# HeewoongNoh/DOSTransformer

Hardware: AMD Instinct MI355X
Metric: crystals/sec training throughput (Phonon DOS, hidden=128) (higher is better)
Workload: dtype f32; 1 GPU; phonon_h128_b64: phonon DOSTransformer layers=3 transformer=2 hidden=128, 64 crystals/GPU, full train step (fwd+loss+bwd+AdamW), 8 distinct pre-collated HBM-resident batches; global_batch=64, parallelism=dp1, launch=replay

## Files before the change

### dostransformer_amd/_lib.py

```python
from __future__ import annotations

import ctypes as C
import os
from typing import Optional

_HERE = os.path.dirname(os.path.abspath(__file__))


def from_environ(name: str, default: str = "") -> str:
    return os.environ.get(name, default)


LIB_PATH = from_environ("DOSX_LIB") or os.path.join(_HERE, "csrc", "libdosx.so")

c_float_p = C.POINTER(C.c_float)
c_int_p = C.POINTER(C.c_int32)
BIG = 1 << 30


class DosxUnavailable(RuntimeError):
    pass


class DosxError(RuntimeError):
# ... 42 lines not shown
        ("pro_gamma", C.c_void_p), ("pro_beta", C.c_void_p), ("pro_alpha", C.c_void_p), ("pro_stats", C.c_void_p),
        ("slab", C.c_void_p), ("slab_bias", C.c_void_p),
        ("nsplit", C.c_int32), ("accumulate", C.c_int32),
        ("dst", C.c_void_p), ("dst_bias", C.c_void_p), ("counters", C.c_void_p), ("ldd", C.c_int32),
    ]


class ReduceJob(C.Structure):
    _fields_ = [("src", C.c_void_p), ("dst", C.c_void_p), ("nsplit", C.c_int32), ("stride", C.c_int32),
                ("count", C.c_int32), ("accumulate", C.c_int32)]


class Attn(C.Structure):
    _fields_ = [
        ("Sq", C.c_int32), ("Bq", C.c_int32), ("Nk", C.c_int32), ("Bk", C.c_int32), ("H", C.c_int32),
        ("q_stride_s", C.c_int32), ("q_stride_b", C.c_int32), ("flags", C.c_int32),
        ("x", C.c_void_p), ("kvhat", C.c_void_p), ("gamma0", C.c_void_p), ("beta0", C.c_void_p),
        ("out", C.c_void_p), ("probs", C.c_void_p), ("qstats", C.c_void_p), ("out_stats", C.c_void_p),
        ("dout", C.c_void_p), ("dx", C.c_void_p), ("dscores", C.c_void_p), ("dkvhat", C.c_void_p),
        ("dkv_accumulate", C.c_int32),
        ("partials_q", C.c_void_p), ("partials_kv", C.c_void_p), ("drop_mask", C.c_void_p), ("dkv_part", C.c_void_p), ("dkv_cnt", C.c_void_p),
        ("ln1_gamma", C.c_void_p), ("ln1_beta", C.c_void_p), ("ln1_out", C.c_void_p),
        ("key_ptr", C.c_void_p),
    ]


class FfnBwd(C.Structure):
    _fields_ = [
        ("M", C.c_int32), ("H", C.c_int32),
        ("dy", C.c_void_p), ("lddy", C.c_int32),
        ("h", C.c_void_p), ("ldh", C.c_int32),
        ("x", C.c_void_p), ("ldx", C.c_int32),
        ("stats", C.c_void_p),
        ("gamma", C.c_void_p),
        ("w1", C.c_void_p), ("w2", C.c_void_p),
        ("dh", C.c_void_p), ("lddh", C.c_int32),
        ("dx", C.c_void_p), ("lddx", C.c_int32),
        ("partials", C.c_void_p), ("partial_ld", C.c_int32),
        ("fin_gamma", C.c_void_p), ("fin_xhat", C.c_void_p), ("fin_rstd", C.c_void_p),
        ("fin_dy", C.c_void_p),
        ("fin_ddos", C.c_void_p), ("fin_w", C.c_void_p), ("fin_beta", C.c_void_p),
        ("fin_S", C.c_int32), ("fin_Bq", C.c_int32),
        ("att_x", C.c_void_p), ("att_ldxin", C.c_int32),
        ("att_kvhat", C.c_void_p), ("att_gamma0", C.c_void_p), ("att_beta0", C.c_void_p),
        ("att_probs", C.c_void_p), ("att_qstats", C.c_void_p), ("att_mask", C.c_void_p),
        ("att_dxin", C.c_void_p), ("att_lddxin", C.c_int32),
        ("att_partials_q", C.c_void_p), ("att_partials_kv", C.c_void_p), ("att_dkv_part", C.c_void_p), ("att_dkv_cnt", C.c_void_p),
        ("att_dkvhat", C.c_void_p), ("att_dkv_accumulate", C.c_int32),
        ("att_Nk", C.c_int32), ("att_Bk", C.c_int32), ("att_Bq", C.c_int32), ("att_Sq", C.c_int32), ("att_qs", C.c_int32), ("att_qb", C.c_int32),
    ]


class Ffn(C.Structure):
    _fields_ = [
        ("M", C.c_int32), ("H", C.c_int32),
        ("x", C.c_void_p), ("ldx", C.c_int32),
        ("stats", C.c_void_p),
        ("gamma", C.c_void_p), ("beta", C.c_void_p),
        ("w1", C.c_void_p), ("b1", C.c_void_p),
        ("w2", C.c_void_p), ("b2", C.c_void_p),
        ("h", C.c_void_p), ("ldh", C.c_int32),
        ("out", C.c_void_p), ("ldo", C.c_int32),
        ("fin_gamma", C.c_void_p), ("fin_beta", C.c_void_p),
        ("fin_xhat", C.c_void_p), ("fin_rstd", C.c_void_p),
        ("fin_w", C.c_void_p), ("fin_b", C.c_void_p), ("fin_dos", C.c_void_p),
        ("fin_S", C.c_int32), ("fin_Bq", C.c_int32),
        ("att_kvhat", C.c_void_p), ("att_gamma0", C.c_void_p), ("att_beta0", C.c_void_p), ("att_mask", C.c_void_p),
        ("att_probs", C.c_void_p), ("att_qstats", C.c_void_p), ("att_x1", C.c_void_p), ("att_st1", C.c_void_p),
        ("att_Nk", C.c_int32), ("att_Bk", C.c_int32), ("att_Bq", C.c_int32), ("att_Sq", C.c_int32),
        ("att_qs", C.c_int32), ("att_qb", C.c_int32), ("att_ldx1", C.c_int32), ("att_aligned", C.c_int32),
        ("att_key_ptr", C.c_void_p),
    ]
# ... 349 lines not shown
```

### dostransformer_amd/csrc/ffn.hip

```cpp
#include <stdlib.h>

#include "common.h"
#include "mma16.h"

typedef int v4i32 __attribute__((ext_vector_type(4)));

#ifdef DOSX_STAMPS
__device__ unsigned long long dosx_ffn_stamp_buf[64];
extern "C" int dosx_debug_read_ffn_stamps(unsigned long long* host64) {
  return (int)hipMemcpyFromSymbol(host64, HIP_SYMBOL(dosx_ffn_stamp_buf), sizeof(unsigned long long) * 64);
}
#define FSTAMP(slot) do { if (threadIdx.x == 0 && blockIdx.x == 0) dosx_ffn_stamp_buf[(slot)] = __builtin_amdgcn_s_memtime(); } while (0)
#define FSTAMP_S(slot) do { if (threadIdx.x == 256 && blockIdx.x == 0) dosx_ffn_stamp_buf[32 + (slot)] = __builtin_amdgcn_s_memtime(); } while (0)
#else
#define FSTAMP(slot) do { } while (0)
#define FSTAMP_S(slot) do { } while (0)
#endif

namespace {

constexpr int FBN = 128;

__device__ __forceinline__ void ffn_att_row(const DosxFfn& a, float* __restrict__ Xs, const int LDX, const int lr, const int m0,
                                            const int lane) {
// ... 606 lines not shown
  ffn_fwd_body<HALF, KB, ATT>(a, sm);
}

constexpr int FFN_MULTI_MAX = 2;
struct FfnMulti {
  DosxFfn d[FFN_MULTI_MAX];
  int n;
};
template <bool HALF, int KB, int ATT>
__global__ __launch_bounds__(512) void ffn_fwd_multi_kernel(const FfnMulti A) {
  DOSX_SET_MAIN_PRIO();
  extern __shared__ __align__(16) float sm[];
  ffn_fwd_body<HALF, KB, ATT>(A.d[0], sm);
  asm volatile("s_waitcnt vmcnt(0)" ::: "memory");
  __syncthreads();
  ffn_fwd_body<HALF, KB, ATT>(A.d[1], sm);
}


struct AttBwdSm {
  float *Os, *Ds, *Ql, *Sp, *Ks, *Sc, *Ss, *Ps2, *Pp;
};

__device__ __forceinline__ void ffn_dkv_reduce(const DosxFfnBwd& a, const int nqt, const int bk, float* __restrict__ Pp, const int tid) {
  const int lane = tid & 63, q16 = lane & 15, slot = tid >> 4;
  const int H = a.H, Nk = a.att_Nk, rep = a.att_Bq / a.att_Bk, ngroups = (Nk + 15) / 16;
  const int np = rep * nqt;
  const UDiv dnqt(nqt);
  const size_t pstride = (size_t)Nk * H;
  const __amdgpu_buffer_rsrc_t rP = __builtin_amdgcn_make_buffer_rsrc((void*)a.att_dkv_part, 0, 0x7fffffff, 0x00020000);
  float4 g0[2], d[2][2], kh[2][2], d0[2][2];
  bool jv[2];
  size_t krow[2];
#pragma unroll
  for (int k = 0; k < 2; ++k) g0[k] = ld4(a.att_gamma0 + ((q16 * 4 + 64 * k) < H ? (q16 * 4 + 64 * k) : 0));
#pragma unroll
  for (int p = 0; p < 2; ++p) {
    const int j = slot + 32 * p;
    jv[p] = j < Nk;
    krow[p] = ((size_t)(jv[p] ? j : 0) * a.att_Bk + bk) * H;
#pragma unroll
    for (int k = 0; k < 2; ++k) {
      const int c = q16 * 4 + 64 * k, cc = c < H ? c : 0;
      kh[p][k] = ld4(a.att_kvhat + krow[p] + cc);
      d0[p][k] = a.att_dkv_accumulate ? ld4(a.att_dkvhat + krow[p] + cc) : f4zero();
      d[p][k] = f4zero();
    }
  }
  for (int p0 = 0; p0 < np; p0 += 4) {
    float4 v[2][4][2];
#pragma unroll
    for (int p = 0; p < 2; ++p)
#pragma unroll
      for (int u = 0; u < 4; ++u) {
        const int pi = min(p0 + u, np - 1), i = dnqt.div(pi), t = pi - i * nqt;
        const size_t off = ((size_t)(bk + i * a.att_Bk) * nqt + t) * pstride + (size_t)(jv[p] ? slot + 32 * p : 0) * H;
#pragma unroll
        for (int k = 0; k < 2; ++k) {
          const int c = q16 * 4 + 64 * k;
          v[p][u][k] = __builtin_bit_cast(float4, __builtin_amdgcn_raw_buffer_load_b128(rP, (uint32_t)((off + (c < H ? c : 0)) * 4), 0, 16));
        }
      }
#pragma unroll
    for (int p = 0; p < 2; ++p)
#pragma unroll
      for (int u = 0; u < 4; ++u)
        if (p0 + u < np) {
#pragma unroll
          for (int k = 0; k < 2; ++k) d[p][k] = f4add(d[p][k], v[p][u][k]);
        }
  }
#pragma unroll
  for (int p = 0; p < 2; ++p)
#pragma unroll
    for (int k = 0; k < 2; ++k) {
      const int c = q16 * 4 + 64 * k;
      float4 pg = f4zero(), pb = f4zero();
      if (jv[p] && c < H) {
        pg = make_float4(d[p][k].x * kh[p][k].x, d[p][k].y * kh[p][k].y, d[p][k].z * kh[p][k].z, d[p][k].w * kh[p][k].w);
        pb = d[p][k];
        st4(a.att_dkvhat + krow[p] + c, make_float4(d[p][k].x * g0[k].x + d0[p][k].x, d[p][k].y * g0[k].y + d0[p][k].y,
                                                    d[p][k].z * g0[k].z + d0[p][k].z, d[p][k].w * g0[k].w + d0[p][k].w));
      }
      st4(Pp + (slot + 32 * p) * 256 + c, pg);
      st4(Pp + (slot + 32 * p) * 256 + 128 + c, pb);
    }
  __syncthreads();
  const UDiv dH(H), d2H(2 * H);
  for (int o = tid; o < ngroups * 2 * H; o += 512) {
    const int grp = d2H.div(o), c = o - grp * 2 * H;
    const int hi = dH.div(c), col = hi * 128 + (c - hi * H);
    float t = 0.f;
#pragma unroll
    for (int sl = 0; sl < 16; ++sl) t += Pp[(grp * 16 + sl) * 256 + col];
    a.att_partials_kv[((size_t)bk * ngroups + grp) * 2 * H + c] = t;
  }
}

struct AttBwdRegs {
  float4 g0[2], b0[2], xr[2], kr[4];
  float mean, rstd, pr[4], mk[4];
};
template <int R>
__device__ __forceinline__ void ffn_att_bwd_prefetch(const DosxFfnBwd& a, AttBwdRegs& q, const int al_s0, const int al_bq, const int tid) {
  const int H = a.H, lane = tid & 63, wave = tid >> 6, q16 = lane & 15, g4 = lane >> 4;
  const int Nk = a.att_Nk, NkP = (Nk + 15) & ~15, Sq = a.att_Sq, bk = al_bq % a.att_Bk;
  const int lr = wave * 4 + g4;
  const int s = min(al_s0 + (lr < R ? lr : 0), Sq - 1);
  const size_t orow = (size_t)s * a.att_Bq + al_bq;
  const float* xrow = a.att_x + ((size_t)s * a.att_qs + (size_t)al_bq * a.att_qb) * a.att_ldxin;
#pragma unroll
  for (int k = 0; k < 2; ++k) {
    const int c = q16 * 4 + 64 * k, cc = c < H ? c : 0;
    q.g0[k] = ld4(a.att_gamma0 + cc); q.b0[k] = ld4(a.att_beta0 + cc);
    q.xr[k] = c < H ? ld4(xrow + c) : f4zero();
  }
  q.mean = a.att_qstats[2 * orow]; q.rstd = a.att_qstats[2 * orow + 1];
  const size_t prow_ = ((size_t)al_bq * Sq + s) * Nk;
#pragma unroll
// ... 34 lines not shown
  const float mean = q.mean, rstd = q.rstd;
#pragma unroll
  for (int jj = 0; jj < 4; ++jj) { pr[jj] = q.pr[jj]; mk[jj] = q.mk[jj]; }
  {
    const int h4 = H >> 2;
    const UDiv dh4(h4);
#pragma unroll
    for (int i = 0; i < 4; ++i) {
      const int e = tid + 512 * i, j = dh4.div(e), c = (e - j * h4) * 4;
      if (e < NkP * h4) st4(L.Ks + j * LDK + c, q.kr[i]);
    }
  }
  FSTAMP(17);
  float cq = 0.f;
  if (rowok) {
    float t = 0.f;
#pragma unroll
    for (int k = 0; k < 2; ++k) {
      go[k] = f4zero();
      if (!on[k]) continue;
      go[k] = ld4(L.Os + lr * LDK + q16 * 4 + 64 * k);
      st4(L.Ds + lr * LDK + q16 * 4 + 64 * k, make_float4(go[k].x * g0[k].x, go[k].y * g0[k].y, go[k].z * g0[k].z, go[k].w * g0[k].w));
      t += (go[k].x * b0[k].x + go[k].y * b0[k].y) + (go[k].z * b0[k].z + go[k].w * b0[k].w);
    }
    if (a.att_mask) cq = row16_sum(t);
  }
  FSTAMP(18);
  __syncthreads();
  FSTAMP(19);
  const int nctS = NkP >> 4, njobsS = (R / 16) * nctS;
  int KS = njobsS >= 8 ? 1 : (njobsS >= 4 ? 2 : 4);
  while (KS > 1 && (H % (16 * KS)) != 0) KS >>= 1;
  const int klen = H / KS;
  const UDiv dKS(KS);
  for (int unit = wave; unit < njobsS * KS; unit += 8) {
    const int job = dKS.div(unit), kq = unit - job * KS;
    const int rt = job >= nctS ? job / nctS : 0, ct = job - rt * nctS;
    const f32x4 acc = mma_kk<8>(L.Ds + (16 * rt + l15) * LDK + kq * klen + 4 * g4, L.Ks + (16 * ct + l15) * LDK + kq * klen + 4 * g4, klen >> 4);
    float* Sq_ = kq == 0 ? L.Sc : L.Sp + (kq - 1) * R * 68;
#pragma unroll
    for (int i = 0; i < 4; ++i) Sq_[(16 * rt + 4 * g4 + i) * 68 + 16 * ct + l15] = acc[i];
  }
  FSTAMP(20);
  __syncthreads();
  if (rowok) {
    float dp[4], dot = 0.f;
// ... 2 lines not shown
      const int j = q16 + 16 * jj;
      float t = 0.f;
      if (j < Nk) {
        t = L.Sc[lr * 68 + j];
        for (int kq = 1; kq < KS; ++kq) t += L.Sp[(kq - 1) * R * 68 + lr * 68 + j];
      }
      if (a.att_mask) t = (t + cq) * mk[jj];
      if (j < Nk) dot += pr[jj] * t;
      dp[jj] = t;
    }
    dot = row16_sum(dot);
#pragma unroll
    for (int jj = 0; jj < 4; ++jj) {
      const int j = q16 + 16 * jj;
      if (j >= NkP) continue;
      const bool v = j < Nk && rv;
      L.Ss[lr * 68 + j] = v ? pr[jj] * (dp[jj] - dot) * scale : 0.f;
      L.Ps2[lr * 68 + j] = v ? pr[jj] * mk[jj] : 0.f;
    }
  }
  FSTAMP(21);
  __syncthreads();
  {
    const int nct = H >> 4, njobs = (R / 16) * nct;
    const UDiv dnct(nct);
    for (int job = wave; job < njobs; job += 8) {
      const int rt = dnct.div(job), ct = job - rt * nct;
      const f32x4 acc = mma_kn<4>(L.Ss + (16 * rt + l15) * 68 + 4 * g4, L.Ks + (4 * g4) * LDK + 16 * ct + l15, LDK, NkP >> 4);
#pragma unroll
      for (int i = 0; i < 4; ++i) L.Ds[(16 * rt + 4 * g4 + i) * LDK + 16 * ct + l15] = acc[i];
    }
  }
  FSTAMP(22);
  __syncthreads();
  FSTAMP(23);
  {
    float4 pg[2] = {f4zero(), f4zero()}, pb[2] = {f4zero(), f4zero()};
    if (rowok) {
      float4 d[2], xh[2];
      float s1 = 0.f, s2 = 0.f;
#pragma unroll
      for (int k = 0; k < 2; ++k) {
        d[k] = f4zero(); xh[k] = f4zero();
        if (!(on[k] && rv)) continue;
        float4 dd = ld4(L.Ds + lr * LDK + q16 * 4 + 64 * k);
        dd = make_float4(dd.x * g0[k].x, dd.y * g0[k].y, dd.z * g0[k].z, dd.w * g0[k].w);
        const float4 xv = xr[k];
        const float4 h = make_float4((xv.x - mean) * rstd, (xv.y - mean) * rstd, (xv.z - mean) * rstd, (xv.w - mean) * rstd);
        d[k] = dd; xh[k] = h;
        pg[k] = make_float4(dd.x * h.x, dd.y * h.y, dd.z * h.z, dd.w * h.w);
        pb[k] = dd;
        const float4 dh = make_float4(dd.x * g0[k].x, dd.y * g0[k].y, dd.z * g0[k].z, dd.w * g0[k].w);
        s1 += (dh.x + dh.y) + (dh.z + dh.w);
        s2 += (dh.x * h.x + dh.y * h.y) + (dh.z * h.z + dh.w * h.w);
      }
      s1 = row16_sum(s1) * invH; s2 = row16_sum(s2) * invH;
#pragma unroll
      for (int k = 0; k < 2; ++k) {
        if (!on[k]) continue;
        const float4 dd = d[k], h = xh[k];
        if (rv)
          st4(a.att_dxin + orow * a.att_lddxin + q16 * 4 + 64 * k,
              make_float4(rstd * (dd.x * g0[k].x - s1 - h.x * s2) + go[k].x, rstd * (dd.y * g0[k].y - s1 - h.y * s2) + go[k].y,
                          rstd * (dd.z * g0[k].z - s1 - h.z * s2) + go[k].z, rstd * (dd.w * g0[k].w - s1 - h.w * s2) + go[k].w));
        st4(L.Ql + lr * LDK + q16 * 4 + 64 * k,
            rv ? make_float4(h.x * g0[k].x + b0[k].x, h.y * g0[k].y + b0[k].y, h.z * g0[k].z + b0[k].z, h.w * g0[k].w + b0[k].w)
               : f4zero());
      }
    }
    const int slot = wave * 4 + g4;
#pragma unroll
    for (int k = 0; k < 2; ++k) {
      const int c = q16 * 4 + 64 * k;
      st4(L.Pp + slot * 256 + c, pg[k]);
      st4(L.Pp + slot * 256 + 128 + c, pb[k]);
    }
  }
  __syncthreads();
  {
    float* prow = a.att_partials_q + ((size_t)al_bq * nqt + tile) * 2 * H;
    for (int c = tid; c < 2 * H; c += 512) {
      const int hi = c >= H ? 1 : 0, o = hi * 128 + (c - hi * H);
      float t = 0.f;
#pragma unroll
      for (int sl = 0; sl < 32; ++sl) t += L.Pp[sl * 256 + o];
      prow[c] = t;
    }
  }
  FSTAMP(24);
  {
    float* part = a.att_dkv_part + ((size_t)al_bq * nqt + tile) * (size_t)Nk * H;
    const int nct = H >> 4, njobs = nctS * nct;
    const UDiv dnct(nct);
    for (int job = wave; job < njobs; job += 8) {
      const int jt = dnct.div(job), ct = job - jt * nct;
      f32x4 acc = {0.f, 0.f, 0.f, 0.f}, acc2 = {0.f, 0.f, 0.f, 0.f};
#pragma unroll
      for (int kk = 0; kk < R; kk += 16) {
        const float* pa = L.Ps2 + (kk + 4 * g4) * 68 + 16 * jt + l15;
        const float* sa = L.Ss + (kk + 4 * g4) * 68 + 16 * jt + l15;
        const float* b1 = L.Os + (kk + 4 * g4) * LDK + 16 * ct + l15;
        const float* b2 = L.Ql + (kk + 4 * g4) * LDK + 16 * ct + l15;
#pragma unroll
        for (int i = 0; i < 4; ++i) {
          acc = __builtin_amdgcn_mfma_f32_16x16x4f32(pa[i * 68], b1[i * LDK], acc, 0, 0, 0);
          acc2 = __builtin_amdgcn_mfma_f32_16x16x4f32(sa[i * 68], b2[i * LDK], acc2, 0, 0, 0);
        }
      }
#pragma unroll
      for (int i = 0; i < 4; ++i) {
        const int j = 16 * jt + 4 * g4 + i, col = 16 * ct + l15;
        if (j < Nk) __hip_atomic_store(part + (size_t)j * H + col, acc[i] + acc2[i], __ATOMIC_RELAXED, __HIP_MEMORY_SCOPE_AGENT);
      }
    }
  }
  FSTAMP(25);
  asm volatile("s_waitcnt vmcnt(0)" ::: "memory");
  __syncthreads();
  FSTAMP(26);
  int* flag = reinterpret_cast<int*>(sm);
  const int arrivers = (a.att_Bq / a.att_Bk) * nqt;
  if (tid == 0) *flag = dosx_ticket(a.att_dkv_cnt + bk);
  __syncthreads();
  const bool last = *flag == arrivers - 1;
  __syncthreads();
  FSTAMP(27);
  if (last) {
    __builtin_amdgcn_fence(__ATOMIC_ACQUIRE, "wavefront");
    ffn_dkv_reduce(a, nqt, bk, sm, tid);
    if (tid == 0) __hip_atomic_store(a.att_dkv_cnt + bk, 0, __ATOMIC_RELAXED, __HIP_MEMORY_SCOPE_AGENT);
    FSTAMP(28);
  }
}

constexpr int BLDW = FBN + 4;

#ifndef DOSX_FFN_BWD_OCC
#define DOSX_FFN_BWD_OCC 2
#endif
// ... 510 lines not shown
}
extern "C" int dosx_ffn_att_bwd_partial_rows(int Sq, int Bq) { return Bq * ceil_div(Sq, ffn_bwd_att_rows(Sq, Bq)); }
extern "C" int dosx_ffn_att_aligned_rows(int Sq, int Bq) { return (Sq < 1 || Bq < 1) ? 0 : ffn_bwd_att_rows(Sq, Bq); }

extern "C" int dosx_ffn_bwd(const DosxFfnBwd* ap, dosx_stream_t stream) {
  DOSX_CHECK_ARG(ap != nullptr, "dosx_ffn_bwd: null descriptor");
  const DosxFfnBwd& a = *ap;
  if (a.M <= 0) return 0;
  DOSX_CHECK_ARG(dosx_ffn_supported(a.H), "dosx_ffn_bwd: H=%d unsupported (multiple of 32, <= 128)", a.H);
  DOSX_CHECK_ARG((a.dy || a.fin_ddos) && a.h && a.x && a.stats && a.gamma && a.w1 && a.w2 && a.dh && (a.dx || a.att_kvhat) && a.partials, "dosx_ffn_bwd: null operand");
  DOSX_CHECK_ARG((a.lddy & 3) == 0 && (a.ldh & 3) == 0 && (a.ldx & 3) == 0 && (a.lddh & 3) == 0 && (a.lddx & 3) == 0,
                 "dosx_ffn_bwd: leading dimensions must be multiples of 4");
  const int npv = a.fin_gamma ? (a.fin_ddos ? 5 : 4) : 2;
  DOSX_CHECK_ARG(a.partial_ld >= npv * a.H + (a.fin_ddos ? 1 : 0), "dosx_ffn_bwd: partial_ld %d too small for %d column groups", a.partial_ld, npv);
  if (a.fin_gamma) DOSX_CHECK_ARG(a.fin_xhat && a.fin_rstd && a.fin_dy, "dosx_ffn_bwd: final LayerNorm backward needs xhat / rstd / fin_dy");
  if (a.fin_ddos) DOSX_CHECK_ARG(a.fin_gamma && a.fin_beta && a.fin_w && a.fin_S > 0 && a.fin_Bq > 0 && a.fin_S * a.fin_Bq == a.M,
                                 "dosx_ffn_bwd: output-layer backward needs gamma / beta / w and S * Bq == M");
  const long long span = (const char*)a.w1 > (const char*)a.w2 ? (const char*)a.w1 - (const char*)a.w2 : (const char*)a.w2 - (const char*)a.w1;
  DOSX_CHECK_ARG(span + (long long)16 * a.H * a.H < 0x7fffffffLL, "dosx_ffn_bwd: fc1 / fc2 weights more than 2 GiB apart");
  const int H = a.H, H4 = 4 * H;
  const bool att = a.att_kvhat != nullptr;
  if (att) {
    DOSX_CHECK_ARG(dosx_ffn_att_bwd_supported(H, a.att_Nk, a.att_Sq, a.att_Bq) && ffn_chunk(H) == 64, "dosx_ffn_bwd: fused attention backward unsupported for H=%d Nk=%d", H, a.att_Nk);
    DOSX_CHECK_ARG(a.att_x && a.att_gamma0 && a.att_beta0 && a.att_probs && a.att_qstats && a.att_dxin && a.att_partials_q && a.att_partials_kv &&
                       a.att_dkv_part && a.att_dkv_cnt && a.att_dkvhat && a.att_Bk > 0 && a.att_Bq % a.att_Bk == 0 && a.att_Sq * a.att_Bq == a.M &&
                       (a.att_ldxin & 3) == 0 && (a.att_lddxin & 3) == 0 && a.att_qs >= 0 && a.att_qb >= 0,
                   "dosx_ffn_bwd: fused attention backward needs x / gamma0 / beta0 / probs / qstats / dxin / partials / dkv scratch + counters and Sq * Bq == M");
  }
  const bool half = att ? ffn_bwd_att_rows(a.att_Sq, a.att_Bq) == 16 : ffn_bwd_half(a.M);
  const int R = half ? 16 : 32;
  const int kb = ffn_chunk(H);
  size_t fl = (size_t)R * (H + 4) + (size_t)R * (H4 + 4) + 2 * (size_t)kb * (FBN + 4);
  if (att && ffn_att_bwd_floats(H, a.att_Nk, R) > fl) fl = ffn_att_bwd_floats(H, a.att_Nk, R);
  const size_t smem = sizeof(float) * fl;
  static bool attr_set = false;
  if (!attr_set) {
    (void)hipFuncSetAttribute(reinterpret_cast<const void*>(&ffn_bwd_kernel<false, 32>), hipFuncAttributeMaxDynamicSharedMemorySize, 160 * 1024);
    (void)hipFuncSetAttribute(reinterpret_cast<const void*>(&ffn_bwd_kernel<true, 32>), hipFuncAttributeMaxDynamicSharedMemorySize, 160 * 1024);
    (void)hipFuncSetAttribute(reinterpret_cast<const void*>(&ffn_bwd_kernel<false, 64>), hipFuncAttributeMaxDynamicSharedMemorySize, 160 * 1024);
    (void)hipFuncSetAttribute(reinterpret_cast<const void*>(&ffn_bwd_kernel<true, 64>), hipFuncAttributeMaxDynamicSharedMemorySize, 160 * 1024);
    (void)hipFuncSetAttribute(reinterpret_cast<const void*>(&ffn_bwd_kernel<false, 64, 2>), hipFuncAttributeMaxDynamicSharedMemorySize, 160 * 1024);
    (void)hipFuncSetAttribute(reinterpret_cast<const void*>(&ffn_bwd_kernel<true, 64, 2>), hipFuncAttributeMaxDynamicSharedMemorySize, 160 * 1024);
    attr_set = true;
  }
  const dim3 grid(att ? a.att_Bq * ceil_div(a.att_Sq, R) : ceil_div(a.M, R));
  if (att && half) hipLaunchKernelGGL((ffn_bwd_kernel<true, 64, 2>), grid, dim3(512), smem, to_stream(stream), a);
  else if (att) hipLaunchKernelGGL((ffn_bwd_kernel<false, 64, 2>), grid, dim3(512), smem, to_stream(stream), a);
  else if (half && kb == 64) hipLaunchKernelGGL((ffn_bwd_kernel<true, 64>), grid, dim3(512), smem, to_stream(stream), a);
  else if (half) hipLaunchKernelGGL((ffn_bwd_kernel<true, 32>), grid, dim3(512), smem, to_stream(stream), a);
  else if (kb == 64) hipLaunchKernelGGL((ffn_bwd_kernel<false, 64>), grid, dim3(512), smem, to_stream(stream), a);
// ... 5 lines not shown
```

### dostransformer_amd/functional.py

```python
from __future__ import annotations

from typing import Dict, List, Optional, Sequence, Tuple

import torch

from . import ops
from ._lib import Attn, Seg, from_environ
from ._lib import load as _lib_load
from .batch import GraphMeta
from .ops import (ACT_LEAKY, ACT_RELU, EPI_LN, EPI_PRELU_BWD, EPI_PRELU_LN_BWD, EPI_PRELU_LN_BWD_SEG, EPI_RELU_MASK, EPI_ROWLN_BWD, EPI_SEGSUM,
                  PRO_LN_PRELU, PRO_PRELU, PRO_ROWLN, GradSink, rowmap, seg)

Params = Dict[str, torch.Tensor]


def _empty(dev, *shape):
    return ops.alloc(dev, *shape)


def _rows32(m: int) -> int:
    return (m + 31) // 32


class SegList:
# ... 16 lines not shown
    for k, t in P.items():
        v = flat[o:o + t.numel()].view(t.shape)
        v.copy_(t)
        out[k] = v
        o += (t.numel() + 3) // 4 * 4
    return out


_FACTOR_EDGE_WGRAD = True
_FACTOR_MIN_GF = 0.5
_FACTOR_FUSED = True
_EDGE_ONE_LAUNCH = True
_EDGE_ONE_LAUNCH_BWD = True
_FACTOR_LAST = True
_FACTOR_LAST_MIN_GF = 1.3
_FACTOR_HEADS = True
_FACTOR_HEADS_MIN_GF = 1.0
_FUSED_ATT_FFN = True
_ATT_FFN_MAX_ROWS = 4096
_ATT_ALIGNED = True
_ATT_ALIGNED_MAX_WGS = 256
_ATT_ROWS_FIRST = True
_FUSED_ATT_BWD = True
_FFN_MULTI = True
_FUSED_FIN_BWD = True
_FUSED_HEAD_FWD = True
_FFN_BF16X3 = from_environ("DOSX_FFN_BF16X3", "0") == "1"

_TAIL_SPLITS = 32
_MID_HOOK_LATE_MAX_H = 128
_FFN_TAIL_MAX = 2048


def _wgrad_linear(sink: GradSink, G: Params, wkey: str, bkey: Optional[str], M: int, N: int, dy: Seg,
                  segs: Sequence[Seg], keep=(), tail: bool = False, dst: Optional[torch.Tensor] = None, **pro) -> None:
    if wkey not in G:
        return
    K = sum(s.width for s in segs)
    ns = ops.wgrad_splits(M, N, K)
    if tail:
        ns = max(ns, min(_TAIL_SPLITS, max(M // 128, 1)))
    nsc = ops.wgrad_scratch_floats(N, K, ns)
    slab = sink.scratch(nsc) if nsc else None
    slab_b = sink.scratch(ns * ((N + 63) // 64) * 64) if (bkey is not None and ns > 1) else None
    kw = dict(dst=G[wkey] if dst is None else dst, dst_bias=G[bkey] if bkey is not None else None, **pro)
    keep = tuple(keep) + tuple(t for t in pro.values() if isinstance(t, torch.Tensor))
# ... 584 lines not shown
    r32 = _rows32(rows)
    dx = dy
    fused_all = ops.ffn_supported(H)
    last_plain = T > 0 and lay[T - 1][9] is None
    fused = fused_all and last_plain
    fin_fused = None
    fin_keys = (pre + ".layer_norm.weight", pre + ".layer_norm.bias")
    if head is not None:
        assert dy is None and fin is None and head_fused_bwd(H, T)
        hg, hb, hx, hr, hd, hw, fin_keys = head
        dx = _empty(dev, rows, H)
        fin_fused = (hg, hx, hr, dx, hd, hw, hb, Sq, Bq)
    elif fin is not None and fused and _FUSED_FIN_BWD and T > 0 and dy.stride(1) == 1:
        dx = _empty(dev, rows, H)
        fin_fused = (P[pre + ".layer_norm.weight"], fin[0], fin[1], dx)
    elif fin is not None:
        xhat, rstd = fin
        part = sink.scratch(r32, 2 * H)
        dx = _empty(dev, rows, H)
        ops.layernorm_bwd(dy, xhat, rstd, P[pre + ".layer_norm.weight"], dx, part, rows, H)
        sink.add(part, 0, G[pre + ".layer_norm.weight"], r32, 2 * H, H)
        sink.add(part, H, G[pre + ".layer_norm.bias"], r32, 2 * H, H)
    nqt, nkt = (Sq + 31) // 32, (Nk + 31) // 32
    for t in reversed(range(T)):
        lp = f"{pre}.layers.{t}"
        x_in, qs, qb, x1, probs, qstats, st1, h, mask, fm = lay[t]
        g1, b1 = P[lp + ".layer_norms.1.weight"], P[lp + ".layer_norms.1.bias"]
        g0, b0 = P[lp + ".layer_norms.0.weight"], P[lp + ".layer_norms.0.bias"]
        dx_res2 = dx
        if fm is not None and fm[2] is not None:
            dy2 = _empty(dev, rows, H)
            ops.mask_residual(dx, fm[2], None, dy2, None, rows, H)
            dx = dy2
        _wgrad_linear(sink, G, lp + ".fc2.weight", lp + ".fc2.bias", rows, H, seg(dx), [seg(h)], keep=(dx,))
        dh = _empty(dev, rows, 4 * H)
        dx1 = _empty(dev, rows, H)
        pld = 2 * H
        fused = fused_all and fm is None
        small = bool(_lib_load().dosx_attention_pkv_supported(int(Nk), int(H)))
        att_in_ffn = (fused and small and _FUSED_ATT_BWD and ops.ffn_att_bwd_supported(H, Nk, Sq, Bq)
                      and ops.ffn_att_bwd_partial_rows(Sq, Bq) <= _ATT_ALIGNED_MAX_WGS)
        att_bwd_args = None
        if att_in_ffn:
            nqt_al = ops.ffn_att_bwd_partial_rows(Sq, Bq) // Bq
            npart_a = Bq * nqt_al + Bk * ((Nk + 15) // 16)
            part_a = sink.scratch(npart_a, 2 * H)
            dxin_a = _empty(dev, rows, H)
            kvp_a = sink.scratch(Bq * nqt_al * Nk, H)
            att_bwd_args = dict(x=x_in, kvhat=kvhat, gamma0=g0, beta0=b0, probs=probs, qstats=qstats, mask=mask, dxin=dxin_a,
                                partials_q=part_a.data_ptr(), partials_kv=part_a.data_ptr() + 4 * Bq * nqt_al * 2 * H, dkv_part=kvp_a,
                                dkv_cnt=ops.COUNTERS.take(dev, Bk), dkvhat=dkvhat, accumulate=0 if (dkv_fresh and t == T - 1) else 1,
                                Nk=Nk, Bk=Bk, Bq=Bq, Sq=Sq, qs=qs, qb=qb)
        if fused:
            rgp = ops.ffn_att_bwd_partial_rows(Sq, Bq) if att_in_ffn else ops.ffn_bwd_partial_rows(rows)
            with_fin = fin_fused is not None and t == T - 1
            pld = (5 * H + 4 if head is not None else 4 * H) if with_fin else 2 * H
            part = sink.scratch(rgp, pld)
            ops.ffn_bwd(rows, H, dy if with_fin else dx, h, x1, st1, g1, P[lp + ".fc1.weight"], P[lp + ".fc2.weight"], dh,
                        None if att_in_ffn else dx1, part, fin=fin_fused if with_fin else None, att=att_bwd_args)
            if with_fin:
                sink.add(part, 2 * H, G[fin_keys[0]], rgp, pld, H)
                sink.add(part, 3 * H, G[fin_keys[1]], rgp, pld, H)
                if head is not None:
                    sink.add(part, 4 * H, G[fin_keys[2]], rgp, pld, H)
                    sink.add(part, 5 * H, G[fin_keys[3]], rgp, pld, 1)
        else:
            if _bf16x3_ok(rows, 4 * H, H) and dx.is_contiguous():
                ops.gemm_bf16x3(dx, P[lp + ".fc2.weight"], dh, w_layout=1, mask=h)
            else:
                ops.gemm(rows, 4 * H, [seg(dx)], P[lp + ".fc2.weight"], dh, w_layout=1, epi=EPI_RELU_MASK, aux=h)
            if fm is not None and fm[1] is not None:
                ops.mask_residual(dh, fm[1], None, dh, None, rows, 4 * H)
        _wgrad_linear(sink, G, lp + ".fc1.weight", lp + ".fc1.bias", rows, 4 * H, seg(dh), [seg(x1)], keep=(dh,),
                      pro=PRO_ROWLN, pro_gamma=g1, pro_beta=b1, pro_stats=st1)
        if not fused:
# ... 645 lines not shown
```

### dostransformer_amd/ops.py

```python
from __future__ import annotations

import ctypes as C
from typing import List, Optional, Sequence, Tuple

import numpy as np
import torch

from . import _lib
from ._lib import Ffn, BIG, Attn, Gemm, ReduceJob, RowMap, Seg, Wgrad

PRO_NONE, PRO_PRELU, PRO_LN_PRELU, PRO_ROWLN = 0, 1, 2, 3
EPI_BIAS_ACT, EPI_LN, EPI_PRELU_LN_BWD, EPI_RELU_MASK, EPI_ROWLN_BWD, EPI_PRELU_BWD, EPI_SEGSUM, EPI_PRELU_LN_BWD_SEG = 0, 1, 2, 3, 4, 5, 6, 7
ACT_NONE, ACT_RELU, ACT_LEAKY = 0, 1, 2


class _KernelTimer:

    def __init__(self):
        self.enabled = False
        self.records = []

    def reset(self, enabled: bool):
        self.enabled = enabled
        self.records = []
# ... 413 lines not shown
    if dy is not None:
        a.dy, a.lddy = dy.data_ptr(), int(dy.stride(0))
    else:
        a.lddy = int(fin[3].stride(0))
    a.h, a.ldh = h.data_ptr(), int(h.stride(0))
    a.x, a.ldx = x.data_ptr(), int(x.stride(0))
    a.stats, a.gamma = stats.data_ptr(), gamma.data_ptr()
    a.w1, a.w2 = w1.data_ptr(), w2.data_ptr()
    a.dh, a.lddh = dh.data_ptr(), int(dh.stride(0))
    if dx is not None:
        a.dx, a.lddx = dx.data_ptr(), int(dx.stride(0))
    a.partials, a.partial_ld = partials.data_ptr(), int(partials.stride(0))
    nk_att = 0
    if att is not None:
        a.att_x, a.att_ldxin = att["x"].data_ptr(), int(att["x"].stride(0))
        a.att_kvhat, a.att_gamma0, a.att_beta0 = att["kvhat"].data_ptr(), att["gamma0"].data_ptr(), att["beta0"].data_ptr()
        a.att_probs, a.att_qstats, a.att_mask = att["probs"].data_ptr(), att["qstats"].data_ptr(), _p(att.get("mask"))
        a.att_dxin, a.att_lddxin = att["dxin"].data_ptr(), int(att["dxin"].stride(0))
        a.att_partials_q, a.att_partials_kv = att["partials_q"], att["partials_kv"]
        a.att_dkv_part, a.att_dkv_cnt = att["dkv_part"].data_ptr(), att["dkv_cnt"]
        a.att_dkvhat, a.att_dkv_accumulate = att["dkvhat"].data_ptr(), int(att["accumulate"])
        a.att_Nk, a.att_Bk, a.att_Bq, a.att_Sq = int(att["Nk"]), int(att["Bk"]), int(att["Bq"]), int(att["Sq"])
        a.att_qs, a.att_qb = int(att["qs"]), int(att["qb"])
        nk_att = a.att_Nk
    _call("dosx_ffn_bwd", C.byref(a), _stream(),
          w=lambda: (f"ffn_bwd[H{H}{',att' if nk_att else ''}]", "ffn_bwd_kernel", "mfma", 16.0 * M * H * H + 10.0 * M * nk_att * H))


MLP_LN_MAX_ROWS = 4096
MLP_LN_MAX_KN = 256 * 256
MLP_LN_MAX_KN_FWD = 512 * 512


def mlp_ln_supported(M: int, K: int, NH: int, NO: int) -> bool:
    return 0 < M <= MLP_LN_MAX_ROWS and K * NH <= MLP_LN_MAX_KN and bool(_lib.load().dosx_mlp_ln_supported(int(K), int(NH), int(NO)))


def mlp_ln_fwd_supported(M: int, K: int, NH: int, NO: int) -> bool:
    return 0 < M <= MLP_LN_MAX_ROWS and K * NH <= MLP_LN_MAX_KN_FWD and bool(_lib.load().dosx_mlp_ln_supported(int(K), int(NH), int(NO)))


MLP_LN_CS_MAX_WGS = 512


def mlp_ln_cs(M: int, K: int, NH: int, NO: int) -> bool:
    return bool(M > 0 and _lib.load().dosx_mlp_ln_cs_supported(int(K), int(NH), int(NO))
# ... 1093 lines not shown
```

### include/dosx.h

```cpp
#ifndef DOSX_H
#define DOSX_H

#include <stddef.h>
#include <stdint.h>

#ifdef __cplusplus
extern "C" {
#endif

typedef void* dosx_stream_t;

typedef struct DosxRowMap {
  int32_t d, m, c, off;
  const int32_t* idx;
} DosxRowMap;

typedef struct DosxSeg {
  const float* p;
  int32_t ld;
  int32_t width;
  DosxRowMap map;
} DosxSeg;

enum {
// ... 241 lines not shown
  const float* x; int32_t ldx;
  const float* stats;
  const float* gamma; const float* beta;
  const float* w1; const float* b1;
  const float* w2; const float* b2;
  float* h; int32_t ldh;
  float* out; int32_t ldo;
  const float* fin_gamma; const float* fin_beta;
  float* fin_xhat; float* fin_rstd;
  const float* fin_w; const float* fin_b; float* fin_dos;
  int32_t fin_S, fin_Bq;
  const float* att_kvhat; const float* att_gamma0; const float* att_beta0; const float* att_mask;
  float* att_probs; float* att_qstats; float* att_x1; float* att_st1;
  int32_t att_Nk, att_Bk, att_Bq, att_Sq, att_qs, att_qb, att_ldx1;
  int32_t att_aligned;
  const int32_t* att_key_ptr;
} DosxFfn;
int dosx_ffn_supported(int H);
int dosx_ffn_att_supported(int H, int Nk);
int dosx_ffn_att_aligned_supported(int H, int Nk);
int dosx_ffn_fwd(const DosxFfn* a, dosx_stream_t stream);
int dosx_ffn_fwd_multi(const DosxFfn* descs, int n, dosx_stream_t stream);

typedef struct DosxFfnBwd {
  int32_t M, H;
  const float* dy; int32_t lddy;
  const float* h; int32_t ldh;
  const float* x; int32_t ldx;
  const float* stats;
  const float* gamma;
  const float* w1; const float* w2;
  float* dh; int32_t lddh;
  float* dx; int32_t lddx;
  float* partials; int32_t partial_ld;
  const float* fin_gamma; const float* fin_xhat; const float* fin_rstd;
  float* fin_dy;
  const float* fin_ddos; const float* fin_w; const float* fin_beta;
  int32_t fin_S, fin_Bq;
  const float* att_x; int32_t att_ldxin;
  const float* att_kvhat; const float* att_gamma0; const float* att_beta0;
  const float* att_probs; const float* att_qstats; const float* att_mask;
  float* att_dxin; int32_t att_lddxin;
  float* att_partials_q; float* att_partials_kv; float* att_dkv_part; int32_t* att_dkv_cnt;
  float* att_dkvhat; int32_t att_dkv_accumulate;
  int32_t att_Nk, att_Bk, att_Bq, att_Sq, att_qs, att_qb;
} DosxFfnBwd;
int dosx_ffn_bwd_partial_rows(int M);
int dosx_ffn_att_bwd_supported(int H, int Nk, int Sq, int Bq);
int dosx_ffn_att_bwd_partial_rows(int Sq, int Bq);
int dosx_ffn_att_aligned_rows(int Sq, int Bq);
int dosx_ffn_bwd(const DosxFfnBwd* a, dosx_stream_t stream);

typedef struct DosxEdgeEnc {
  int32_t E, H;
  const float* vec;
  float inv_rmax;
  const float* w0; const float* b0;
  const float* alpha;
  const float* w2; const float* b2;
  float* attr; float* z;
  float* out; int32_t ldo;
} DosxEdgeEnc;
int dosx_edge_enc_supported(int H);
int dosx_edge_enc_fwd(const DosxEdgeEnc* a, dosx_stream_t stream);

typedef struct DosxHeadsBwd {
  int32_t S, B, H;
  const float* dkvs; const float* kvs; const float* rstd;
// ... 313 lines not shown
```

Before: 61450 crystals/s.

## Defer attention key-gradient reduction into the next layer's fused FFN backward

The fused FFN+attention backward for one transformer layer can now only publish its per-tile key/value gradient partials and skip the cross-workgroup reduction. The next layer's launch then reduces the deferred set along with its own, carrying the running dkvhat in registers and writing it once. Separately, the dK/dV partial MFMA jobs are merged into the same job loop as the dQ matmul, and the normalized-query staging is moved earlier so both can run together. The aim is to drop one counter/synchronisation tail and one dkvhat read-modify-write per layer pair. In exchange, the reducing launch does more serial work and there are more descriptor fields to validate.

Result: no change. 61700 crystals/s, median of 2 (+0.4%).

```diff
diff --git a/dostransformer_amd/_lib.py b/dostransformer_amd/_lib.py
--- a/dostransformer_amd/_lib.py
+++ b/dostransformer_amd/_lib.py
@@ -88,6 +88,16 @@
         ("partials_q", C.c_void_p), ("partials_kv", C.c_void_p), ("drop_mask", C.c_void_p), ("dkv_part", C.c_void_p), ("dkv_cnt", C.c_void_p),
         ("ln1_gamma", C.c_void_p), ("ln1_beta", C.c_void_p), ("ln1_out", C.c_void_p),
         ("key_ptr", C.c_void_p),
+    ]
+
+
+FFN_MAX_DEFER = 3
+
+
+class FfnDefer(C.Structure):
+    _fields_ = [
+        ("dkv_part", C.c_void_p), ("gamma0", C.c_void_p), ("partials_kv", C.c_void_p),
+        ("Bq", C.c_int32), ("nqt", C.c_int32), ("fresh", C.c_int32),
     ]
 
 
@@ -114,6 +124,8 @@
         ("att_partials_q", C.c_void_p), ("att_partials_kv", C.c_void_p), ("att_dkv_part", C.c_void_p), ("att_dkv_cnt", C.c_void_p),
         ("att_dkvhat", C.c_void_p), ("att_dkv_accumulate", C.c_int32),
         ("att_Nk", C.c_int32), ("att_Bk", C.c_int32), ("att_Bq", C.c_int32), ("att_Sq", C.c_int32), ("att_qs", C.c_int32), ("att_qb", C.c_int32),
+        ("att_dkv_publish_only", C.c_int32), ("att_n_defer", C.c_int32),
+        ("att_defer", FfnDefer * FFN_MAX_DEFER),
     ]
 
 
diff --git a/dostransformer_amd/csrc/ffn.hip b/dostransformer_amd/csrc/ffn.hip
--- a/dostransformer_amd/csrc/ffn.hip
+++ b/dostransformer_amd/csrc/ffn.hip
@@ -652,31 +652,29 @@
   float *Os, *Ds, *Ql, *Sp, *Ks, *Sc, *Ss, *Ps2, *Pp;
 };
 
-__device__ __forceinline__ void ffn_dkv_reduce(const DosxFfnBwd& a, const int nqt, const int bk, float* __restrict__ Pp, const int tid) {
+struct DkvRows {
+  float4 kh[2][2], run[2][2];
+  bool jv[2];
+};
+__device__ __forceinline__ void ffn_dkv_reduce_set(const DosxFfnBwd& a, DkvRows& R, const float* part, const float* g0p, float* pkv, const int Bq,
+                                                   const int nqt, const bool fresh, const bool sync_first, const int bk, float* __restrict__ Pp,
+                                                   const int tid) {
   const int lane = tid & 63, q16 = lane & 15, slot = tid >> 4;
-  const int H = a.H, Nk = a.att_Nk, rep = a.att_Bq / a.att_Bk, ngroups = (Nk + 15) / 16;
-  const int np = rep * nqt;
+  const int H = a.H, Nk = a.att_Nk, ngroups = (Nk + 15) / 16;
+  const size_t pstride = (size_t)Nk * H;
+  const int np = (Bq / a.att_Bk) * nqt;
   const UDiv dnqt(nqt);
-  const size_t pstride = (size_t)Nk * H;
-  const __amdgpu_buffer_rsrc_t rP = __builtin_amdgcn_make_buffer_rsrc((void*)a.att_dkv_part, 0, 0x7fffffff, 0x00020000);
-  float4 g0[2], d[2][2], kh[2][2], d0[2][2];
-  bool jv[2];
-  size_t krow[2];
-#pragma unroll
-  for (int k = 0; k < 2; ++k) g0[k] = ld4(a.att_gamma0 + ((q16 * 4 + 64 * k) < H ? (q16 * 4 + 64 * k) : 0));
-#pragma unroll
-  for (int p = 0; p < 2; ++p) {
-    const int j = slot + 32 * p;
-    jv[p] = j < Nk;
-    krow[p] = ((size_t)(jv[p] ? j : 0) * a.att_Bk + bk) * H;
-#pragma unroll
-    for (int k = 0; k < 2; ++k) {
-      const int c = q16 * 4 + 64 * k, cc = c < H ? c : 0;
-      kh[p][k] = ld4(a.att_kvhat + krow[p] + cc);
-      d0[p][k] = a.att_dkv_accumulate ? ld4(a.att_dkvhat + krow[p] + cc) : f4zero();
+  const __amdgpu_buffer_rsrc_t rP = __builtin_amdgcn_make_buffer_rsrc((void*)part, 0, 0x7fffffff, 0x00020000);
+  float4 g0[2], d[2][2];
+#pragma unroll
+  for (int k = 0; k < 2; ++k) g0[k] = ld4(g0p + ((q16 * 4 + 64 * k) < H ? (q16 * 4 + 64 * k) : 0));
+#pragma unroll
+  for (int p = 0; p < 2; ++p)
+#pragma unroll
+    for (int k = 0; k < 2; ++k) {
       d[p][k] = f4zero();
-    }
-  }
+      if (fresh) R.run[p][k] = f4zero();
+    }
   for (int p0 = 0; p0 < np; p0 += 4) {
     float4 v[2][4][2];
 #pragma unroll
@@ -684,7 +682,7 @@
 #pragma unroll
       for (int u = 0; u < 4; ++u) {
         const int pi = min(p0 + u, np - 1), i = dnqt.div(pi), t = pi - i * nqt;
-        const size_t off = ((size_t)(bk + i * a.att_Bk) * nqt + t) * pstride + (size_t)(jv[p] ? slot + 32 * p : 0) * H;
+        const size_t off = ((size_t)(bk + i * a.att_Bk) * nqt + t) * pstride + (size_t)(R.jv[p] ? slot + 32 * p : 0) * H;
 #pragma unroll
         for (int k = 0; k < 2; ++k) {
           const int c = q16 * 4 + 64 * k;
@@ -700,17 +698,19 @@
           for (int k = 0; k < 2; ++k) d[p][k] = f4add(d[p][k], v[p][u][k]);
         }
   }
+  if (sync_first) __syncthreads();
 #pragma unroll
   for (int p = 0; p < 2; ++p)
 #pragma unroll
     for (int k = 0; k < 2; ++k) {
       const int c = q16 * 4 + 64 * k;
       float4 pg = f4zero(), pb = f4zero();
-      if (jv[p] && c < H) {
-        pg = make_float4(d[p][k].x * kh[p][k].x, d[p][k].y * kh[p][k].y, d[p][k].z * kh[p][k].z, d[p][k].w * kh[p][k].w);
+      if (R.jv[p] && c < H) {
+        const float4 kh = R.kh[p][k], d0 = R.run[p][k];
+        pg = make_float4(d[p][k].x * kh.x, d[p][k].y * kh.y, d[p][k].z * kh.z, d[p][k].w * kh.w);
         pb = d[p][k];
-        st4(a.att_dkvhat + krow[p] + c, make_float4(d[p][k].x * g0[k].x + d0[p][k].x, d[p][k].y * g0[k].y + d0[p][k].y,
-                                                    d[p][k].z * g0[k].z + d0[p][k].z, d[p][k].w * g0[k].w + d0[p][k].w));
+        R.run[p][k] = make_float4(d[p][k].x * g0[k].x + d0.x, d[p][k].y * g0[k].y + d0.y,
+                                  d[p][k].z * g0[k].z + d0.z, d[p][k].w * g0[k].w + d0.w);
       }
       st4(Pp + (slot + 32 * p) * 256 + c, pg);
       st4(Pp + (slot + 32 * p) * 256 + 128 + c, pb);
@@ -723,8 +723,43 @@
     float t = 0.f;
 #pragma unroll
     for (int sl = 0; sl < 16; ++sl) t += Pp[(grp * 16 + sl) * 256 + col];
-    a.att_partials_kv[((size_t)bk * ngroups + grp) * 2 * H + c] = t;
-  }
+    pkv[((size_t)bk * ngroups + grp) * 2 * H + c] = t;
+  }
+}
+__device__ __forceinline__ void ffn_dkv_reduce(const DosxFfnBwd& a, const int nqt, const int bk, float* __restrict__ Pp, const int tid) {
+  const int lane = tid & 63, q16 = lane & 15, slot = tid >> 4;
+  const int H = a.H, nd = a.att_n_defer;
+  DkvRows R;
+  size_t krow[2];
+  const bool load0 = nd > 0 ? a.att_defer[0].fresh == 0 : a.att_dkv_accumulate != 0;
+#pragma unroll
+  for (int p = 0; p < 2; ++p) {
+    const int j = slot + 32 * p;
+    R.jv[p] = j < a.att_Nk;
+    krow[p] = ((size_t)(R.jv[p] ? j : 0) * a.att_Bk + bk) * H;
+#pragma unroll
+    for (int k = 0; k < 2; ++k) {
+      const int c = q16 * 4 + 64 * k, cc = c < H ? c : 0;
+      R.kh[p][k] = ld4(a.att_kvhat + krow[p] + cc);
+      R.run[p][k] = load0 ? ld4(a.att_dkvhat + krow[p] + cc) : f4zero();
+    }
+  }
+#define DOSX_DKV_DEFERRED(I)                                                                                                      \
+  if (nd > I) ffn_dkv_reduce_set(a, R, a.att_defer[I].dkv_part, a.att_defer[I].gamma0, a.att_defer[I].partials_kv, a.att_defer[I].Bq, \
+                                 a.att_defer[I].nqt, a.att_defer[I].fresh != 0, I > 0, bk, Pp, tid)
+  DOSX_DKV_DEFERRED(0);
+  DOSX_DKV_DEFERRED(1);
+  DOSX_DKV_DEFERRED(2);
+#undef DOSX_DKV_DEFERRED
+  static_assert(DOSX_FFN_MAX_DEFER == 3, "one DOSX_DKV_DEFERRED per table entry");
+  ffn_dkv_reduce_set(a, R, a.att_dkv_part, a.att_gamma0, a.att_partials_kv, a.att_Bq, nqt, a.att_dkv_accumulate == 0, nd > 0, bk, Pp, tid);
+#pragma unroll
+  for (int p = 0; p < 2; ++p)
+#pragma unroll
+    for (int k = 0; k < 2; ++k) {
+      const int c = q16 * 4 + 64 * k;
+      if (R.jv[p] && c < H) st4(a.att_dkvhat + krow[p] + c, R.run[p][k]);
+    }
 }
 
 struct AttBwdRegs {
@@ -805,6 +840,11 @@
       go[k] = ld4(L.Os + lr * LDK + q16 * 4 + 64 * k);
       st4(L.Ds + lr * LDK + q16 * 4 + 64 * k, make_float4(go[k].x * g0[k].x, go[k].y * g0[k].y, go[k].z * g0[k].z, go[k].w * g0[k].w));
       t += (go[k].x * b0[k].x + go[k].y * b0[k].y) + (go[k].z * b0[k].z + go[k].w * b0[k].w);
+      const float4 xv = xr[k];
+      const float4 h = make_float4((xv.x - mean) * rstd, (xv.y - mean) * rstd, (xv.z - mean) * rstd, (xv.w - mean) * rstd);
+      st4(L.Ql + lr * LDK + q16 * 4 + 64 * k,
+          rv ? make_float4(h.x * g0[k].x + b0[k].x, h.y * g0[k].y + b0[k].y, h.z * g0[k].z + b0[k].z, h.w * g0[k].w + b0[k].w)
+             : f4zero());
     }
     if (a.att_mask) cq = row16_sum(t);
   }
@@ -853,13 +893,36 @@
   FSTAMP(21);
   __syncthreads();
   {
-    const int nct = H >> 4, njobs = (R / 16) * nct;
+    float* part = a.att_dkv_part + ((size_t)al_bq * nqt + tile) * (size_t)Nk * H;
+    const int nct = H >> 4, nkv = nctS * nct, njobs = nkv + (R / 16) * nct;
     const UDiv dnct(nct);
     for (int job = wave; job < njobs; job += 8) {
-      const int rt = dnct.div(job), ct = job - rt * nct;
-      const f32x4 acc = mma_kn<4>(L.Ss + (16 * rt + l15) * 68 + 4 * g4, L.Ks + (4 * g4) * LDK + 16 * ct + l15, LDK, NkP >> 4);
-#pragma unroll
-      for (int i = 0; i < 4; ++i) L.Ds[(16 * rt + 4 * g4 + i) * LDK + 16 * ct + l15] = acc[i];
+      if (job < nkv) {
+        const int jt = dnct.div(job), ct = job - jt * nct;
+        f32x4 acc = {0.f, 0.f, 0.f, 0.f}, acc2 = {0.f, 0.f, 0.f, 0.f};
+#pragma unroll
+        for (int kk = 0; kk < R; kk += 16) {
+          const float* pa = L.Ps2 + (kk + 4 * g4) * 68 + 16 * jt + l15;
+          const float* sa = L.Ss + (kk + 4 * g4) * 68 + 16 * jt + l15;
+          const float* b1 = L.Os + (kk + 4 * g4) * LDK + 16 * ct + l15;
+          const float* b2 = L.Ql + (kk + 4 * g4) * LDK + 16 * ct + l15;
+#pragma unroll
+          for (int i = 0; i < 4; ++i) {
+            acc = __builtin_amdgcn_mfma_f32_16x16x4f32(pa[i * 68], b1[i * LDK], acc, 0, 0, 0);
+            acc2 = __builtin_amdgcn_mfma_f32_16x16x4f32(sa[i * 68], b2[i * LDK], acc2, 0, 0, 0);
+          }
+        }
+#pragma unroll
+        for (int i = 0; i < 4; ++i) {
+          const int j = 16 * jt + 4 * g4 + i, col = 16 * ct + l15;
+          if (j < Nk) __hip_atomic_store(part + (size_t)j * H + col, acc[i] + acc2[i], __ATOMIC_RELAXED, __HIP_MEMORY_SCOPE_AGENT);
+        }
+      } else {
+        const int jq = job - nkv, rt = dnct.div(jq), ct = jq - rt * nct;
+        const f32x4 acc = mma_kn<4>(L.Ss + (16 * rt + l15) * 68 + 4 * g4, L.Ks + (4 * g4) * LDK + 16 * ct + l15, LDK, NkP >> 4);
+#pragma unroll
+        for (int i = 0; i < 4; ++i) L.Ds[(16 * rt + 4 * g4 + i) * LDK + 16 * ct + l15] = acc[i];
+      }
     }
   }
   FSTAMP(22);
@@ -894,9 +957,6 @@
           st4(a.att_dxin + orow * a.att_lddxin + q16 * 4 + 64 * k,
               make_float4(rstd * (dd.x * g0[k].x - s1 - h.x * s2) + go[k].x, rstd * (dd.y * g0[k].y - s1 - h.y * s2) + go[k].y,
                           rstd * (dd.z * g0[k].z - s1 - h.z * s2) + go[k].z, rstd * (dd.w * g0[k].w - s1 - h.w * s2) + go[k].w));
-        st4(L.Ql + lr * LDK + q16 * 4 + 64 * k,
-            rv ? make_float4(h.x * g0[k].x + b0[k].x, h.y * g0[k].y + b0[k].y, h.z * g0[k].z + b0[k].z, h.w * g0[k].w + b0[k].w)
-               : f4zero());
       }
     }
     const int slot = wave * 4 + g4;
@@ -919,33 +979,8 @@
     }
   }
   FSTAMP(24);
-  {
-    float* part = a.att_dkv_part + ((size_t)al_bq * nqt + tile) * (size_t)Nk * H;
-    const int nct = H >> 4, njobs = nctS * nct;
-    const UDiv dnct(nct);
-    for (int job = wave; job < njobs; job += 8) {
-      const int jt = dnct.div(job), ct = job - jt * nct;
-      f32x4 acc = {0.f, 0.f, 0.f, 0.f}, acc2 = {0.f, 0.f, 0.f, 0.f};
-#pragma unroll
-      for (int kk = 0; kk < R; kk += 16) {
-        const float* pa = L.Ps2 + (kk + 4 * g4) * 68 + 16 * jt + l15;
-        const float* sa = L.Ss + (kk + 4 * g4) * 68 + 16 * jt + l15;
-        const float* b1 = L.Os + (kk + 4 * g4) * LDK + 16 * ct + l15;
-        const float* b2 = L.Ql + (kk + 4 * g4) * LDK + 16 * ct + l15;
-#pragma unroll
-        for (int i = 0; i < 4; ++i) {
-          acc = __builtin_amdgcn_mfma_f32_16x16x4f32(pa[i * 68], b1[i * LDK], acc, 0, 0, 0);
-          acc2 = __builtin_amdgcn_mfma_f32_16x16x4f32(sa[i * 68], b2[i * LDK], acc2, 0, 0, 0);
-        }
-      }
-#pragma unroll
-      for (int i = 0; i < 4; ++i) {
-        const int j = 16 * jt + 4 * g4 + i, col = 16 * ct + l15;
-        if (j < Nk) __hip_atomic_store(part + (size_t)j * H + col, acc[i] + acc2[i], __ATOMIC_RELAXED, __HIP_MEMORY_SCOPE_AGENT);
-      }
-    }
-  }
   FSTAMP(25);
+  if (a.att_dkv_publish_only) return;
   asm volatile("s_waitcnt vmcnt(0)" ::: "memory");
   __syncthreads();
   FSTAMP(26);
@@ -1502,10 +1537,19 @@
   const bool att = a.att_kvhat != nullptr;
   if (att) {
     DOSX_CHECK_ARG(dosx_ffn_att_bwd_supported(H, a.att_Nk, a.att_Sq, a.att_Bq) && ffn_chunk(H) == 64, "dosx_ffn_bwd: fused attention backward unsupported for H=%d Nk=%d", H, a.att_Nk);
-    DOSX_CHECK_ARG(a.att_x && a.att_gamma0 && a.att_beta0 && a.att_probs && a.att_qstats && a.att_dxin && a.att_partials_q && a.att_partials_kv &&
-                       a.att_dkv_part && a.att_dkv_cnt && a.att_dkvhat && a.att_Bk > 0 && a.att_Bq % a.att_Bk == 0 && a.att_Sq * a.att_Bq == a.M &&
+    const bool pub = a.att_dkv_publish_only != 0;
+    DOSX_CHECK_ARG(a.att_x && a.att_gamma0 && a.att_beta0 && a.att_probs && a.att_qstats && a.att_dxin && a.att_partials_q && (pub || a.att_partials_kv) &&
+                       a.att_dkv_part && (pub || a.att_dkv_cnt) && (pub || a.att_dkvhat) && a.att_Bk > 0 && a.att_Bq % a.att_Bk == 0 && a.att_Sq * a.att_Bq == a.M &&
                        (a.att_ldxin & 3) == 0 && (a.att_lddxin & 3) == 0 && a.att_qs >= 0 && a.att_qb >= 0,
                    "dosx_ffn_bwd: fused attention backward needs x / gamma0 / beta0 / probs / qstats / dxin / partials / dkv scratch + counters and Sq * Bq == M");
+    DOSX_CHECK_ARG(a.att_n_defer >= 0 && a.att_n_defer <= DOSX_FFN_MAX_DEFER, "dosx_ffn_bwd: att_n_defer=%d outside 0 .. %d", a.att_n_defer, DOSX_FFN_MAX_DEFER);
+    DOSX_CHECK_ARG(!(pub && a.att_n_defer > 0), "dosx_ffn_bwd: a publish-only launch cannot reduce deferred sets (att_n_defer=%d)", a.att_n_defer);
+    for (int i = 0; i < a.att_n_defer; ++i) {
+      const DosxFfnDefer& d = a.att_defer[i];
+      DOSX_CHECK_ARG(d.dkv_part && d.gamma0 && d.partials_kv, "dosx_ffn_bwd: deferred set %d has a null pointer", i);
+      DOSX_CHECK_ARG(d.Bq > 0 && d.Bq % a.att_Bk == 0 && d.nqt > 0, "dosx_ffn_bwd: deferred set %d: Bq=%d must be a positive multiple of att_Bk=%d and nqt=%d positive",
+                     i, d.Bq, a.att_Bk, d.nqt);
+    }
   }
   const bool half = att ? ffn_bwd_att_rows(a.att_Sq, a.att_Bq) == 16 : ffn_bwd_half(a.M);
   const int R = half ? 16 : 32;
diff --git a/dostransformer_amd/functional.py b/dostransformer_amd/functional.py
--- a/dostransformer_amd/functional.py
+++ b/dostransformer_amd/functional.py
@@ -62,6 +62,7 @@
 _ATT_ALIGNED_MAX_WGS = 256
 _ATT_ROWS_FIRST = True
 _FUSED_ATT_BWD = True
+_DEFER_DKV = True
 _FFN_MULTI = True
 _FUSED_FIN_BWD = True
 _FUSED_HEAD_FWD = True
@@ -692,6 +693,12 @@
         sink.add(part, 0, G[pre + ".layer_norm.weight"], r32, 2 * H, H)
         sink.add(part, H, G[pre + ".layer_norm.bias"], r32, 2 * H, H)
     nqt, nkt = (Sq + 31) // 32, (Nk + 31) // 32
+    small = bool(_lib_load().dosx_attention_pkv_supported(int(Nk), int(H)))
+
+    def att_in_ffn_at(t_):
+        return bool(fused_all and lay[t_][9] is None and small and _FUSED_ATT_BWD and ops.ffn_att_bwd_supported(H, Nk, Sq, Bq)
+                    and ops.ffn_att_bwd_partial_rows(Sq, Bq) <= _ATT_ALIGNED_MAX_WGS)
+    deferred = []
     for t in reversed(range(T)):
         lp = f"{pre}.layers.{t}"
         x_in, qs, qb, x1, probs, qstats, st1, h, mask, fm = lay[t]
@@ -707,9 +714,7 @@
         dx1 = _empty(dev, rows, H)
         pld = 2 * H
         fused = fused_all and fm is None
-        small = bool(_lib_load().dosx_attention_pkv_supported(int(Nk), int(H)))
-        att_in_ffn = (fused and small and _FUSED_ATT_BWD and ops.ffn_att_bwd_supported(H, Nk, Sq, Bq)
-                      and ops.ffn_att_bwd_partial_rows(Sq, Bq) <= _ATT_ALIGNED_MAX_WGS)
+        att_in_ffn = att_in_ffn_at(t)
         att_bwd_args = None
         if att_in_ffn:
             nqt_al = ops.ffn_att_bwd_partial_rows(Sq, Bq) // Bq
@@ -719,8 +724,15 @@
             kvp_a = sink.scratch(Bq * nqt_al * Nk, H)
             att_bwd_args = dict(x=x_in, kvhat=kvhat, gamma0=g0, beta0=b0, probs=probs, qstats=qstats, mask=mask, dxin=dxin_a,
                                 partials_q=part_a.data_ptr(), partials_kv=part_a.data_ptr() + 4 * Bq * nqt_al * 2 * H, dkv_part=kvp_a,
-                                dkv_cnt=ops.COUNTERS.take(dev, Bk), dkvhat=dkvhat, accumulate=0 if (dkv_fresh and t == T - 1) else 1,
+                                dkvhat=dkvhat, accumulate=0 if (dkv_fresh and t == T - 1) else 1,
                                 Nk=Nk, Bk=Bk, Bq=Bq, Sq=Sq, qs=qs, qb=qb)
+            if _DEFER_DKV and not deferred and t > 0 and att_in_ffn_at(t - 1):
+                att_bwd_args.update(publish_only=True, dkv_cnt=None)
+                deferred = [dict(dkv_part=kvp_a, gamma0=g0, partials_kv=att_bwd_args["partials_kv"], Bq=Bq, nqt=nqt_al,
+                                 fresh=1 - att_bwd_args["accumulate"])]
+            else:
+                att_bwd_args.update(defer=deferred, dkv_cnt=ops.COUNTERS.take(dev, Bk))
+                deferred = []
         if fused:
             rgp = ops.ffn_att_bwd_partial_rows(Sq, Bq) if att_in_ffn else ops.ffn_bwd_partial_rows(rows)
             with_fin = fin_fused is not None and t == T - 1
diff --git a/dostransformer_amd/ops.py b/dostransformer_amd/ops.py
--- a/dostransformer_amd/ops.py
+++ b/dostransformer_amd/ops.py
@@ -459,6 +459,15 @@
         a.att_dkvhat, a.att_dkv_accumulate = att["dkvhat"].data_ptr(), int(att["accumulate"])
         a.att_Nk, a.att_Bk, a.att_Bq, a.att_Sq = int(att["Nk"]), int(att["Bk"]), int(att["Bq"]), int(att["Sq"])
         a.att_qs, a.att_qb = int(att["qs"]), int(att["qb"])
+        a.att_dkv_publish_only = int(bool(att.get("publish_only", False)))
+        sets = att.get("defer") or ()
+        if len(sets) > _lib.FFN_MAX_DEFER:
+            raise ValueError(f"ffn_bwd: {len(sets)} deferred key-gradient sets, at most {_lib.FFN_MAX_DEFER}")
+        a.att_n_defer = len(sets)
+        for i, d in enumerate(sets):
+            e = a.att_defer[i]
+            e.dkv_part, e.gamma0, e.partials_kv = d["dkv_part"].data_ptr(), d["gamma0"].data_ptr(), d["partials_kv"]
+            e.Bq, e.nqt, e.fresh = int(d["Bq"]), int(d["nqt"]), int(d["fresh"])
         nk_att = a.att_Nk
     _call("dosx_ffn_bwd", C.byref(a), _stream(),
           w=lambda: (f"ffn_bwd[H{H}{',att' if nk_att else ''}]", "ffn_bwd_kernel", "mfma", 16.0 * M * H * H + 10.0 * M * nk_att * H))
diff --git a/include/dosx.h b/include/dosx.h
--- a/include/dosx.h
+++ b/include/dosx.h
@@ -287,6 +287,14 @@
 int dosx_ffn_fwd(const DosxFfn* a, dosx_stream_t stream);
 int dosx_ffn_fwd_multi(const DosxFfn* descs, int n, dosx_stream_t stream);
 
+#define DOSX_FFN_MAX_DEFER 3
+typedef struct DosxFfnDefer {
+  const float* dkv_part;
+  const float* gamma0;
+  float* partials_kv;
+  int32_t Bq, nqt;
+  int32_t fresh;
+} DosxFfnDefer;
 typedef struct DosxFfnBwd {
   int32_t M, H;
   const float* dy; int32_t lddy;
@@ -309,6 +317,8 @@
   float* att_partials_q; float* att_partials_kv; float* att_dkv_part; int32_t* att_dkv_cnt;
   float* att_dkvhat; int32_t att_dkv_accumulate;
   int32_t att_Nk, att_Bk, att_Bq, att_Sq, att_qs, att_qb;
+  int32_t att_dkv_publish_only, att_n_defer;
+  DosxFfnDefer att_defer[DOSX_FFN_MAX_DEFER];
 } DosxFfnBwd;
 int dosx_ffn_bwd_partial_rows(int M);
 int dosx_ffn_att_bwd_supported(int H, int Nk, int Sq, int Bq);
```
